# matchylabs/matchy

Measured on AMD Instinct MI355X. Metric: log GB/s scanned (matchy match hot path, 100K IoCs), higher is better.
Workload: dtype u8

## Files before the change

matchy_amd/csrc/db_image.cpp:

```cpp
#include "db_image.h"

#include <cstring>

namespace mxy {

namespace {
inline uint32_t rd32(const uint8_t* p) { uint32_t v; memcpy(&v, p, 4); return v; }
inline uint64_t rd64(const uint8_t* p) { uint64_t v; memcpy(&v, p, 8); return v; }

long find_metadata_marker(const uint8_t* d, size_t n) {
    static const uint8_t M[14] = {0xAB, 0xCD, 0xEF, 'M', 'a', 'x', 'M', 'i', 'n', 'd', '.', 'c', 'o', 'm'};
    if (n < 14) return -1;
    size_t start = n > 128 * 1024 ? n - 128 * 1024 : 0;
    long last = -1;
    for (size_t i = start; i + 14 <= n; ++i)
        if (memcmp(d + i, M, 14) == 0) last = (long)i;
    return last;
}
bool meta_uint(const DataValue& m, const char* key, uint64_t& out) {
    auto it = m.map.find(key);
    if (it == m.map.end()) return false;
    const DataValue& v = it->second;
    if (v.type != DataValue::UINT16 && v.type != DataValue::UINT32 && v.type != DataValue::UINT64) return false;
    out = v.u;
// ... 238 lines not shown
    }
    v4_start = 0;
    if (ip_version == 6) {
        uint32_t node = 0;
        for (int k = 0; k < 96; ++k) {
            uint32_t rec = out[node].x;
            if (rec < node_count) node = rec;
            else break;
        }
        v4_start = node;
    }
}

void DbImage::build_lit_table(std::vector<LitSlot>& slots, uint32_t& mask) const {
    const uint8_t* lh = bytes.data() + lh_off;
    size_t live = 0;
    for (uint32_t i = 0; i < lh_table_size; ++i) live += rd32(lh + lh_table_start + (size_t)i * 16 + 8) != 0xFFFFFFFFu;
    size_t cap = 16;
    while (cap < live * 2) cap <<= 1;
    mask = (uint32_t)(cap - 1);
    slots.assign(cap, LitSlot{0, 0xFFFFFFFFu, 0});
    for (uint32_t i = 0; i < lh_table_size; ++i) {
        const uint8_t* e = lh + lh_table_start + (size_t)i * 16;
        uint32_t so = rd32(e + 8);
        if (so == 0xFFFFFFFFu) continue;
        if ((size_t)so + 2 > lh_strings_size) continue;
        uint64_t h = rd64(e);
        uint32_t s = (uint32_t)(h ^ (h >> 32)) & mask;
        while (slots[s].str_off != 0xFFFFFFFFu) s = (s + 1) & mask;
        slots[s] = LitSlot{h, so, rd32(e + 12)};
    }
}

void DbImage::build_lit2pat(std::vector<uint32_t>& off, std::vector<uint32_t>& ids) const {
    off.assign(1, 0);
    ids.clear();
    if (!has_glob) return;
    const uint8_t* pg = bytes.data() + pg_off;
    uint32_t map_off = rd32(pg + 96), map_cnt = rd32(pg + 100);
    if (map_cnt == 0 || map_off == 0 || (size_t)map_off + 24 > pg_len) return;
    const uint8_t* a = pg + map_off;
    size_t alen = pg_len - map_off;
    if (memcmp(a, "ACLH", 4) != 0) return;
    uint32_t table_size = rd32(a + 12), pstart = rd32(a + 16);
    if (24 + (size_t)table_size * 16 > alen) return;
// ... 118 lines not shown
```

matchy_amd/csrc/engine.cpp:

```cpp
#include "engine.h"
#include "batch_reader.h"
#include "distinct.h"
#include "extract_render_core.h"
#include "render_core.h"
#include "tally.h"
#include "unicode_lower.h"

#include <dlfcn.h>

#include <algorithm>
#include <chrono>
#include <cstdio>
#include <cstdlib>
#include <cstring>
#include <stdexcept>
#include <unordered_set>

#include "domain_prefilter.h"
#include "hashes.h"

namespace mxy {

void check_launch(const char* kernel) {
    const hipError_t e = hipGetLastError();
// ... 239 lines not shown
            for (uint32_t wv : bm) set += (uint64_t)__builtin_popcount(wv);
            view.ip_bm24_permille = (uint32_t)(set * 1000 / ((uint64_t)bm.size() * 32));
            view.ip_bm24_any = set ? 1u : 0u;
        }
        bytes_uploaded += bm.size() * 4;
    }
    if (img.has_literal) {
        std::vector<LitSlot> slots;
        uint32_t mask;
        img.build_lit_table(slots, mask);
        lit_slots.upload(slots);
        const uint8_t* pool = img.bytes.data() + img.lh_off + img.lh_strings_offset;
        std::vector<uint8_t> pv(pool, pool + img.lh_strings_size);
        lit_pool.upload(pv);
        {
            size_t bits = (size_t)1 << 22;
            size_t live = 0;
            for (const LitSlot& sl : slots) live += sl.str_off != 0xFFFFFFFFu;
            while (bits < live * 64 && bits < ((size_t)1 << 31)) bits <<= 1;
            std::vector<uint32_t> bm(bits / 32, 0u);
            const uint32_t bmask = (uint32_t)(bits - 1);
            for (const LitSlot& sl : slots) {
                if (sl.str_off == 0xFFFFFFFFu || (size_t)sl.str_off + 2 > pv.size()) continue;
                const size_t kl = (size_t)pv[sl.str_off] | ((size_t)pv[sl.str_off + 1] << 8);
                if ((size_t)sl.str_off + 2 + kl > pv.size()) continue;
                uint64_t lane[4] = {0, 0, 0, 0};
                memcpy(lane, pv.data() + sl.str_off + 2, std::min<size_t>(kl, 32));
                const uint32_t b = name_hash31(lane[0], lane[1], lane[2], lane[3], (uint32_t)kl) & bmask;
                bm[b >> 5] |= 1u << (b & 31);
            }
            lit_bm.upload(bm);
            view.lit_bm = lit_bm.p; view.lit_bm_mask = bmask;
            bytes_uploaded += bm.size() * 4;
        }
        uint32_t max_len = 0;
        for (const LitSlot& sl : slots)
            if (sl.str_off != 0xFFFFFFFFu && (size_t)sl.str_off + 2 <= pv.size()) max_len = std::max<uint32_t>(max_len, (uint32_t)pv[sl.str_off] | ((uint32_t)pv[sl.str_off + 1] << 8));
        view.lit_max_len = max_len;
        view.lit_slots = lit_slots.p; view.lit_mask = mask; view.has_literal = 1;
        view.lit_pool = lit_pool.p; view.lit_pool_size = img.lh_strings_size;
        bytes_uploaded += slots.size() * sizeof(LitSlot) + pv.size();
    }
    if (img.has_glob) {
        const uint8_t* pgp = img.bytes.data() + img.pg_off;
        std::vector<uint8_t> pv(pgp, pgp + img.pg_len);
        pv.resize((pv.size() + 3) & ~(size_t)3, 0);
        pg.upload(pv);
        std::vector<uint32_t> off, ids;
        img.build_lit2pat(off, ids);
        if (ids.empty()) ids.push_back(0);
        lit2pat_off.upload(off);
        lit2pat.upload(ids);
// ... 782 lines not shown
            hh.n_cand_r = std::max(hh.n_cand_r, q.n_cand_r); hh.n_cand_d = std::max(hh.n_cand_d, q.n_cand_d);
            hh.n_dom = std::max(hh.n_dom, q.n_dom);
        }
        hint_ = hh;
    }
    const ScanCounters& c = host_counters_;
    if (c.error & 1) throw HipError{"scan: a candidate matches more than 65535 glob patterns (the hit record counts pattern ids in 16 bits)"};
    if (c.error & 4) throw HipError{"scan: a candidate is longer than 16 MiB (24-bit length field)"};
    if (trace) {
        ScanCounters t = host_slices_.p[0];
        for (int k = 1; k < ns; ++k) {
            const ScanCounters& s = host_slices_.p[k];
            t.n_dom += s.n_dom; t.n_rare += s.n_rare; t.n_rare_dom += s.n_rare_dom; t.n_tok += s.n_tok; t.n_heavy += s.n_heavy; t.n_cand_a += s.n_cand_a;
            t.n_cand += s.n_cand; t.n_hits += s.n_hits; t.n_ids += s.n_ids; t.n_glob_work += s.n_glob_work;
        }
        fprintf(stderr, "[matchy_amd] slices=%d lines=%llu n_dom=%u n_rare=%u+%u n_tok=%u n_heavy=%u n_cand=%u+%u (true %u) n_hits=%u (true %u) n_ids=%u glob_work=%u final=%u\n",
                ns, c.lines, t.n_dom, t.n_rare, t.n_rare_dom, t.n_tok, t.n_heavy, t.n_cand_a, t.n_cand, c.cand_true, t.n_hits, c.hits_true, t.n_ids, t.n_glob_work, c.n_final);
    }
    out.lines = c.lines; out.n_cand = single_ ? c.n_cand : c.cand_true;
    out.n_hits = !last_.lookup ? 0 : (single_ ? c.hits_true : c.n_final + (compact_ ? c.n_c4 : 0u));
    if (profile_) {
        MXY_HIP(hipEventElapsedTime(&timing_.anchor_ms, ev_[0], ev_[1]));
        if (last_forked_) {
            MXY_HIP(hipEventElapsedTime(&timing_.validate_ms, ev_[1], ev_[4]));
            timing_.rare_ms = 0; timing_.lookup_ms = 0;
        } else {
            MXY_HIP(hipEventElapsedTime(&timing_.validate_ms, ev_[1], ev_[2]));
            MXY_HIP(hipEventElapsedTime(&timing_.rare_ms, ev_[2], ev_[3]));
            MXY_HIP(hipEventElapsedTime(&timing_.lookup_ms, ev_[3], ev_[4]));
        }
        MXY_HIP(hipEventElapsedTime(&timing_.total_ms, ev_[0], ev_[4]));
        timing_.slices = ns;
// ... 584 lines not shown
```

matchy_amd/csrc/hashes.h:

```cpp
#pragma once
#include <cstddef>
#include <cstdint>

#if defined(__HIPCC__)
#include <hip/hip_runtime.h>
#define MXY_HD __host__ __device__ inline __attribute__((always_inline))
#else
#define MXY_HD inline
#endif

namespace mxy {

MXY_HD uint64_t rotl64(uint64_t x, int r) { return (x << r) | (x >> (64 - r)); }

template <class Fetch>
MXY_HD uint64_t xxh64_fetch(Fetch f, size_t len, uint64_t seed) {
    const uint64_t P1 = 11400714785074694791ULL, P2 = 14029467366897019727ULL, P3 = 1609587929392839161ULL,
                   P4 = 9650029242287828579ULL, P5 = 2870177450012600261ULL;
    auto rd64 = [&](size_t o) {
        uint64_t v = 0;
        for (int k = 7; k >= 0; --k) v = (v << 8) | (uint64_t)f(o + k);
        return v;
    };
    auto rd32 = [&](size_t o) {
// ... 117 lines not shown
};

MXY_HD uint32_t name_hash31(uint64_t l0, uint64_t l1, uint64_t l2, uint64_t l3, uint32_t n) {
    const uint64_t lane[4] = {l0, l1, l2, l3};
    uint32_t h = n * 0x9E3779B1u + 0x7F4A7C15u;
    for (int k = 0; k < 4; ++k) {
        const int rem = (int)n - 8 * k;
        const uint64_t m = rem >= 8 ? ~0ull : rem <= 0 ? 0ull : ((1ull << (8 * rem)) - 1ull);
        const uint64_t v = lane[k] & m;
        h = (h ^ (uint32_t)v) * 0x85EBCA6Bu; h ^= h >> 15;
        h = (h ^ (uint32_t)(v >> 32)) * 0xC2B2AE35u; h ^= h >> 13;
    }
    h *= 0x27D4EB2Fu; h ^= h >> 16;
    return h;
}

MXY_HD uint64_t fx_u32(uint32_t v) { return rotl64((uint64_t)v * 0xf1357aea2e62a9c5ULL, 26); }

constexpr uint32_t TLD_TAB_BITS = 11;
MXY_HD uint32_t tld_tab_slot(uint32_t lo, uint32_t hi24) { return ((lo ^ (hi24 * 0x9E3779B1u)) * 0x85EBCA6Bu) >> (32 - TLD_TAB_BITS); }

constexpr uint32_t TLD_PFX_BITS = 10;
constexpr uint32_t TLD_PFX_MAX_KEYS = (3u << TLD_PFX_BITS) / 4;
MXY_HD uint32_t tld_pfx_slot(uint32_t lo, uint32_t hi) { return ((lo ^ (hi * 0x9E3779B1u)) * 0x85EBCA6Bu) >> (32 - TLD_PFX_BITS); }

template <class Slot>
MXY_HD bool tld_pfx_has(const Slot* tab, uint32_t lo, uint32_t hi) {
    uint32_t slot = tld_pfx_slot(lo, hi);
    for (;;) {
        const Slot t = tab[slot];
// ... 29 lines not shown
```

matchy_amd/csrc/lookup_kernels.hip:

```cpp
#include <hip/hip_runtime.h>

#include <cstdlib>

#include "hashes.h"
#include "scan_types.h"

#include "device_shared.h"

namespace mxy {


__device__ __forceinline__ uint32_t d_utf8_decode(const uint8_t* s, uint32_t& cp) {
    const uint32_t c = s[0];
    if (c < 0x80) { cp = c; return 1; }
    if (c < 0xE0) { cp = ((c & 0x1Fu) << 6) | (s[1] & 0x3Fu); return 2; }
    if (c < 0xF0) { cp = ((c & 0x0Fu) << 12) | ((s[1] & 0x3Fu) << 6) | (s[2] & 0x3Fu); return 3; }
    cp = ((c & 0x07u) << 18) | ((s[1] & 0x3Fu) << 12) | ((s[2] & 0x3Fu) << 6) | (s[3] & 0x3Fu);
    return 4;
}
__device__ bool d_cp_in_ranges(const uint2* r, uint32_t n, uint32_t cp) {
    uint32_t lo = 0, hi = n;
    while (lo < hi) { const uint32_t mid = (lo + hi) >> 1; if (r[mid].y < cp) lo = mid + 1; else hi = mid; }
    return lo < n && r[lo].x <= cp;
}
// ... 38 lines not shown
                if (lo < db.lc_n && db.lc_map[lo * 3] == cp) {
                    const uint32_t e1 = db.lc_map[lo * 3 + 1];
                    np = e1 & 0xFF; pend = (uint64_t)(e1 >> 8) | ((uint64_t)db.lc_map[lo * 3 + 2] << 24);
                } else {
                    pend = 0; np = a;
                    for (uint32_t k = 0; k < a; ++k) pend |= (uint64_t)s[i + k] << (8 * k);
                }
            }
            i += a;
        }
        b = (uint32_t)pend & 0xFF; pend >>= 8; --np;
        return true;
    }
};

__device__ bool lit_lookup(const DevDb& db, const uint8_t* s0, uint32_t n0, uint32_t& pattern_id) {
    const uint8_t* s = s0;
    uint32_t n = n0;
    bool fold = false, stream = false;
    uint64_t h;
    if (db.ci) {
        uint64_t hi = 0;
        uint32_t k = 0;
        for (; k + 8 <= n0; k += 8) { uint64_t x; __builtin_memcpy(&x, s0 + k, 8); hi |= x; }
        for (; k < n0; ++k) hi |= s0[k];
        if ((hi & 0x8080808080808080ull) == 0) fold = true;
        else stream = true;
    }
    if (stream) {
        LowerStream ls(db, s0, n0);
        Xxh64Stream xs(0);
        uint32_t b;
        n = 0;
        while (ls.next(b)) {
            xs.push(b);
            if (++n > db.lit_max_len) return false;
        }
        h = xs.finish(0);
    } else {
        h = fold ? xxh64<true>(s, n, 0) : xxh64<false>(s, n, 0);
    }
    uint32_t slot = (uint32_t)(h ^ (h >> 32)) & db.lit_mask;
    for (;;) {
        LitSlot e = db.lit_slots[slot];
        if (e.str_off == 0xFFFFFFFFu) return false;
        if (e.hash == h) {
            const uint8_t* q = db.lit_pool + e.str_off;
            uint32_t sl = (uint32_t)q[0] | ((uint32_t)q[1] << 8);
            if (sl == n) {
                uint64_t diff = 0;
                if (stream) {
                    LowerStream ls(db, s0, n0);
                    uint32_t b, k = 0;
                    while (ls.next(b)) { diff |= (uint64_t)(q[2 + k] ^ b); ++k; }
                } else {
                    uint32_t k = 0;
                    for (; k + 8 <= n; k += 8) {
                        uint64_t x, y;
                        __builtin_memcpy(&x, q + 2 + k, 8);
                        __builtin_memcpy(&y, s + k, 8);
                        diff |= x ^ (fold ? ascii_lower8(y) : y);
                    }
                    if (k < n) {
                        if (n >= 8) {
                            uint64_t x, y;
                            __builtin_memcpy(&x, q + 2 + n - 8, 8);
                            __builtin_memcpy(&y, s + n - 8, 8);
                            diff |= x ^ (fold ? ascii_lower8(y) : y);
                        } else {
                            for (; k < n; ++k) diff |= (uint64_t)(q[2 + k] ^ (fold ? ascii_lower1(s[k]) : (uint32_t)s[k]));
                        }
                    }
                }
                if (diff == 0) { pattern_id = e.pattern_id; return true; }
            }
        }
        slot = (slot + 1) & db.lit_mask;
    }
}

__device__ __forceinline__ uint32_t ld32(const uint8_t* p) { return *reinterpret_cast<const uint32_t*>(p); }

__device__ uint32_t ac_transition(const uint8_t* ac, uint32_t ac_len, uint32_t node_off, uint32_t ch) {
    if (node_off + 20 > ac_len) return 0xFFFFFFFFu;
    uint32_t w0 = ld32(ac + node_off);
    uint32_t kind = w0 & 0xFF;
    if (kind == 1) return ((w0 >> 8) & 0xFF) == ch ? ld32(ac + node_off + 12) : 0xFFFFFFFFu;
    if (kind == 2) {
        uint32_t eo = ld32(ac + node_off + 12), cnt = (w0 >> 16) & 0xFF;
        if (eo + cnt * 8 > ac_len) return 0xFFFFFFFFu;
        for (uint32_t i = 0; i < cnt; ++i) {
            uint32_t ec = ac[eo + i * 8];
            if (ec == ch) return ld32(ac + eo + i * 8 + 4);
// ... 407 lines not shown
        }
        if (c.len_type != 0xFFFFFFFFu) {
            uint32_t type = c.len_type >> 24, tl = c.len_type & 0xFFFFFF;
            const uint8_t* text = p.log + c.start;
            h.cand = i; h.start = c.start; h.len_type = c.len_type;
            if (type == IT_IPV4) {
                uint32_t off, pfx;
                if (db.has_ip && trie_v4(db, c.v4, off, pfx)) { h.kind = 2; h.a = off; h.prefix_len = (uint8_t)pfx; emit = true; }
            } else if (type == IT_IPV6) {
                uint16_t seg[8];
                uint32_t off, pfx;
                if (db.has_ip && d_parse_ipv6(text, tl, seg) && trie_v6(db, seg, off, pfx)) { h.kind = 2; h.a = off; h.prefix_len = (uint8_t)pfx; emit = true; }
            } else {
                const bool alnum_tok = type == IT_MD5 || type == IT_SHA1 || type == IT_SHA256 || type == IT_SHA384 || type == IT_SHA512 ||
                                       type == IT_BITCOIN || type == IT_ETHEREUM || type == IT_MONERO;
                if (!db.ac_alnum && alnum_tok) c.pad = CAND_NO_GLOB;
                if (!GLOB && p.ac_filter && p.early_glob && c.pad == CAND_GLOB) {
                } else if (!GLOB && p.ac_filter && (c.pad == CAND_GLOB || (c.pad != CAND_NO_GLOB && (defer_unwalked || ac_touches_output(db, dv, text, tl))))) defer = true;
                else {
                    uint32_t pid = 0xFFFFFFFFu;
                    if (db.has_literal) { uint32_t q; if (lit_lookup(db, text, tl, q)) pid = q; }
                    if constexpr (GLOB) {
                        GlobSetList rs{globs};
                        StarStackFixed stk;
                        glob_find_all(db, dv, text_stage(p.log, p.len, c.start, tl, twin + threadIdx.x * GLOB_WIN_WORDS), outq + threadIdx.x * GLOB_OUTQ, rs, stk);
                        ng = rs.n;
                        spill = rs.over;
                    }
                    if (!spill && (pid != 0xFFFFFFFFu || ng)) { h.kind = 3; h.a = pid; h.n_globs = (uint16_t)ng; emit = true; }
                }
            }
        }
        if (p.direct && !GLOB) {
            if (emit) { pend[pn] = PendRec{h.start, h.len_type, h.a, (uint32_t)h.kind | ((uint32_t)h.prefix_len << 8)}; ++pn; }
            if (__ballot(pn == PEND_RECS)) { pack_pending(p.pk, pn, pend); pn = 0; }
        } else if (p.direct) {
// ... 42 lines not shown
    Hit SH{};
    SH.kind = 0xFF;
    for (uint32_t base = blockIdx.x * blockDim.x; base < n; base += stride) {
        const uint32_t k = base + threadIdx.x;
        Hit h{};
        bool emit = false;
        if (k < n) {
            const uint32_t tagged = p.spill[k], i = tagged & 0x7FFFFFFFu;
            const bool alt = (tagged >> 31) != 0;
            const Candidate c = alt ? (p.cands_alt && i < p.cand_alt_cap ? p.cands_alt[i] : Candidate{0, 0xFFFFFFFFu, 0, 0})
                                    : (i < p.cand_cap ? p.cands[i] : Candidate{0, 0xFFFFFFFFu, 0, 0});
            if (c.len_type != 0xFFFFFFFFu) {
                const uint32_t tl = c.len_type & 0xFFFFFF;
                h.cand = i; h.start = c.start; h.len_type = c.len_type;
                uint32_t pid = 0xFFFFFFFFu;
                if (db.has_literal) { uint32_t q; if (lit_lookup(db, p.log + c.start, tl, q)) pid = q; }
                for (uint32_t w = 0; w < bit_words; ++w) bits[w] = 0;
                GlobSetBitmap rs{bits, db.pattern_count};
                StarStackMem stk{bits + bit_words, (p.spill_words - bit_words) / 2};
                glob_find_all(db, dv, text_stage(p.log, p.len, c.start, tl, twin + threadIdx.x * GLOB_WIN_WORDS), outq + threadIdx.x * GLOB_OUTQ, rs, stk);
                uint32_t ng = rs.n;
                if (rs.over || ng > 0xFFFFu) { atomicOr(&p.counters->error, 1u); ng = 0; }
                if (ng) {
                    const uint32_t io = atomicAdd(&p.counters->n_ids, ng);
                    h.ids_off = io;
                    uint32_t o = io;
                    for (uint32_t w = 0; w < bit_words; ++w)
                        for (uint32_t m = bits[w]; m; m &= m - 1, ++o)
                            if (o < p.ids_cap) p.ids[o] = 32 * w + (uint32_t)__builtin_ctz(m);
                }
                if (pid != 0xFFFFFFFFu || ng) { h.kind = 3; h.a = pid; h.n_globs = (uint16_t)ng; emit = true; }
// ... 102 lines not shown
```

matchy_amd/csrc/scan_types.h:

```cpp
#pragma once
#include <hip/hip_runtime.h>

#include <cstdint>

namespace mxy {

enum ItemType : uint8_t {
    IT_DOMAIN = 0, IT_EMAIL = 1, IT_IPV4 = 2, IT_IPV6 = 3, IT_MD5 = 4, IT_SHA1 = 5, IT_SHA256 = 6,
    IT_SHA384 = 7, IT_SHA512 = 8, IT_BITCOIN = 9, IT_ETHEREUM = 10, IT_MONERO = 11, IT_COUNT = 12
};
enum ExtractFlags : uint32_t {
    EX_DOMAINS = 1, EX_EMAILS = 2, EX_IPV4 = 4, EX_IPV6 = 8, EX_HASHES = 16, EX_BITCOIN = 32, EX_ETHEREUM = 64,
    EX_MONERO = 128, EX_ALL = 255
};

struct Candidate {
    uint32_t start;
    uint32_t len_type;
    uint32_t v4;
    uint32_t pad;
};
constexpr uint32_t CAND_NO_GLOB = 1, CAND_GLOB = 2;

enum RareKind : uint32_t { RARE_V6 = 0, RARE_AT = 1, RARE_TOK = 2, HEAVY_B58 = 3, HEAVY_BECH32 = 4, HEAVY_ETH = 5, HEAVY_XMR = 6, RARE_DOM = 7 };
struct RareAnchor {
    uint32_t pos;
    uint32_t len_kind;
};

struct Hit {
    uint32_t cand;
    uint32_t a;
    uint32_t ids_off;
    uint16_t n_globs;
    uint8_t kind;
    uint8_t prefix_len;
    uint32_t start;
    uint32_t len_type;
};

struct LitSlot { uint64_t hash; uint32_t str_off; uint32_t pattern_id; };
struct PslSlot { uint64_t hash; uint32_t off; uint32_t len; };

struct DevDb {
    const uint2* ip_nodes;
    uint32_t ip_bm24_permille;
    uint32_t ip_bm24_any;
    const uint32_t* ip_bm24;
    const uint2* ip_l1;
    const uint2* ip_l24;
    const uint2* ip_leaf;
    uint32_t node_count;
    uint32_t ip_version;
    uint32_t v4_start_node;
    uint32_t has_ip;
    const LitSlot* lit_slots;
// ... 207 lines not shown
```

matchy_amd/csrc/validate_kernels.hip:

```cpp
#include <hip/hip_runtime.h>

#include <cstdlib>

#include "hashes.h"
#include "scan_types.h"

#include "device_shared.h"
#include "domain_planes.h"

namespace mxy {


struct BackReader {
    const uint8_t* p;
    uint32_t pos;
    uint32_t cb;
    uint32_t k;
    uint64_t cur, nxt;
    __device__ __forceinline__ static uint64_t load8(const uint8_t* a) { uint64_t v; __builtin_memcpy(&v, a, 8); return v; }
    __device__ __forceinline__ void init(const uint8_t* base, uint32_t q) {
        p = base; pos = q; cb = 0; k = 0; cur = 0; nxt = 0;
        if (q >= 16) { cb = q - 8; k = 8; cur = load8(p + cb); nxt = load8(p + cb - 8); }
    }
    __device__ __forceinline__ uint32_t next() {
// ... 761 lines not shown
    auto load_rec = [&](uint32_t i, Rec& r) {
        const uint32_t ic = i < nd ? i : 0u;
        const uint32_t j = p.dom_list[dom_plane_index(ic, 0)];
#pragma unroll
        for (int k = 0; k < 8; ++k) r.c[k] = p.dom_list[dom_plane_index(ic, 1 + k)];
        r.j = i < nd ? j : 0xFFFFFFFFu;
    };
    Rec cur, nxt;
    load_rec(blockIdx.x * blockDim.x + threadIdx.x, cur);
    {
        uint32_t g = cur.j;
#pragma unroll
        for (int k = 0; k < 8; ++k) g ^= cur.c[k];
        asm volatile("" ::"v"(g));
    }
    uint32_t pend_start = 0, pend_lt = 0, pend_word = 0xFFFFFFFFu, pend_bit = 0, n_valid = 0;
    uint32_t pend_sw[SFX ? 4 : 1] = {0}, pend_sb[SFX ? 4 : 1] = {0};
    bool pend = false, pend_over = false;
    uint32_t* sb = strbuf[threadIdx.x];
    auto queue_glob = [&](uint32_t b, uint32_t n) {
        if (!p.glob_work_d) return;
        const uint32_t lane = lane_id();
        const bool g = lane < n && b + lane < p.cand_cap && cw.buf[lane].pad == CAND_GLOB;
        const uint64_t m = __ballot(g);
        if (!m) return;
        uint32_t wb = 0;
        if (lane == 0) wb = atomicAdd(&p.counters->n_glob_work_d, (uint32_t)__popcll(m));
        wb = __builtin_amdgcn_readfirstlane(wb);
        const uint32_t slot = wb + mbcnt64(m);
        if (g && slot < p.glob_work_d_cap) p.glob_work_d[slot] = b + lane;
    };
    auto emit_pending = [&]() {
        if (!p.filter_lit) { cw_dense.append(pend, Candidate{pend_start, pend_lt, 0u, 0u}, p.cands, p.cand_cap, p.n_cand, SC); return; }
        bool lit = (pend_word >> pend_bit) & 1;
        uint32_t flag = 0;
        if constexpr (SFX) {
            bool g = pend_over;
#pragma unroll
            for (int q = 0; q < 4; ++q) g = g || ((pend_sw[q] >> pend_sb[q]) & 1);
            flag = g ? CAND_GLOB : CAND_NO_GLOB;
            lit = lit || g;
        }
        if constexpr (AC) flag = pend_over ? CAND_GLOB : CAND_NO_GLOB;
        if constexpr (AC || SFX) cw.append_then(pend && lit, Candidate{pend_start, pend_lt, 0u, flag}, p.cands, p.cand_cap, p.n_cand, queue_glob);
        else cw.append(pend && lit, Candidate{pend_start, pend_lt, 0u, flag}, p.cands, p.cand_cap, p.n_cand);
    };
    for (uint32_t base = blockIdx.x * blockDim.x; base < nd; base += stride) {
        const uint32_t i = base + threadIdx.x;
        emit_pending();
        pend = false;
        load_rec(i + stride, nxt);
        bool slow = false;
        if (cur.j != 0xFFFFFFFFu) {
            uint32_t s = 0, e = 0;
            int r = 2;
            if (!(cur.j & 0x80000000u)) r = domain_rules(tldtab, db.tld_pfx, p.min_labels, cur.j, cur.c, s, e);
            slow = r == 2;
            if (r == 1) {
                pend_start = s; pend_lt = (e - s) | ((uint32_t)IT_DOMAIN << 24); pend = true;
                pend_word = 0xFFFFFFFFu; pend_bit = 0;
                n_valid += 1;
                if (p.filter_lit) {
                    *reinterpret_cast<uint4*>(sb) = make_uint4(cur.c[0], cur.c[1], cur.c[2], cur.c[3]);
                    *reinterpret_cast<uint4*>(sb + 4) = make_uint4(cur.c[4], cur.c[5], cur.c[6], cur.c[7]);
                    const uint32_t o = 24 - (cur.j - s), n = e - s;
                    const uint32_t i0 = o >> 2, sh = o & 3;
                    uint32_t wd[9];
#pragma unroll
                    for (int k = 0; k < 9; ++k) wd[k] = (i0 + k) < 8 ? sb[(i0 + k) & 7] : 0u;
                    uint64_t ln[4];
#pragma unroll
                    for (int k = 0; k < 4; ++k)
                        ln[k] = (uint64_t)__builtin_amdgcn_alignbyte(wd[2 * k + 1], wd[2 * k], sh) |
                                ((uint64_t)__builtin_amdgcn_alignbyte(wd[2 * k + 2], wd[2 * k + 1], sh) << 32);
                    if (db.ci) {
#pragma unroll
                        for (int k = 0; k < 4; ++k) ln[k] = ascii_lower8(ln[k]);
                    }
                    const uint32_t b = name_hash31(ln[0], ln[1], ln[2], ln[3], n) & db.lit_bm_mask;
                    pend_word = db.lit_bm ? db.lit_bm[b >> 5] : 0u;
                    pend_bit = b & 31;
                    if constexpr (SFX) {
                        const uint64_t fb = 0x0101010101010101ull * db.sfx_first;
                        uint32_t M = 0;
#pragma unroll
                        for (int k = 0; k < 4; ++k) {
                            const uint64_t x = ln[k] ^ fb;
                            const uint64_t z = ~(((x & 0x7F7F7F7F7F7F7F7Full) + 0x7F7F7F7F7F7F7F7Full) | x) & 0x8080808080808080ull;
                            const uint32_t lo = (uint32_t)z >> 7, hi = (uint32_t)(z >> 32) >> 7;
                            M |= ((((lo * 0x01020408u) >> 24) & 0xFu) | ((((hi * 0x01020408u) >> 24) & 0xFu) << 4)) << (8 * k);
                        }
                        M &= n >= 32 ? 0xFFFFFFFFu : ((1u << n) - 1u);
                        pend_over = false;
                        uint32_t dm = db.sfx_dots;
#pragma unroll
                        for (int q = 0; q < 4; ++q) {
// ... 27 lines not shown
                            }
                        }
                    }
                    if constexpr (AC) {
                        uint32_t st = 0, any = 0;
#pragma unroll
                        for (int k = 0; k < 31; ++k) {
                            const uint32_t c = dcls[(uint32_t)(ln[k >> 3] >> (8 * (k & 7))) & 0xFF];
                            if ((uint32_t)k < n) {
                                const uint32_t t = st < dv.lds_states ? drows[st * db.dfa_k + c] : db.dfa[(size_t)st * db.dfa_k + c];
                                st = t & 0x7FFFFFFFu;
                                any |= t;
                            }
                        }
                        pend_over = (any >> 31) != 0;
                        if (pend_over) { pend_word = 0xFFFFFFFFu; pend_bit = 0; }
                    }
                }
            }
        }
        sw.append(slow, RareAnchor{cur.j & 0x7FFFFFFFu, (uint32_t)RARE_DOM}, p.rare_dom, p.rare_dom_cap, &p.counters->n_rare_dom);
        cur = nxt;
    }
    emit_pending();
    if constexpr (AC || SFX) cw.flush_then(p.cands, p.cand_cap, p.n_cand, queue_glob);
    else cw.flush(p.cands, p.cand_cap, p.n_cand);
    cw_dense.pad_rest(p.cands, p.cand_cap, SC);
    sw.flush(p.rare_dom, p.rare_dom_cap, &p.counters->n_rare_dom);
#pragma unroll
    for (int off = 32; off > 0; off >>= 1) n_valid += __shfl_down(n_valid, off);
    if (lane_id() == 0 && n_valid) atomicAdd(&p.counters->cand_true, n_valid);
}

__device__ __forceinline__ bool lit_bm_may_hit(const DevDb& db, const LogView& lg, uint32_t s, uint32_t n, bool ascii) {
    uint64_t l[4] = {0, 0, 0, 0};
    if (s + 32 <= lg.len) {
#pragma unroll
        for (int k = 0; k < 4; ++k) __builtin_memcpy(&l[k], lg.p + s + 8 * k, 8);
    } else {
        for (uint32_t k = 0; k < 32 && s + k < lg.len; ++k) l[k >> 3] |= (uint64_t)lg.p[s + k] << (8 * (k & 7));
    }
    if (db.ci) {
        if (!ascii) {
            if (n > 32) return true;
            uint64_t high = 0;
#pragma unroll
            for (int k = 0; k < 4; ++k) {
                const int rem = (int)n - 8 * k;
                const uint64_t m = rem >= 8 ? ~0ull : (rem <= 0 ? 0ull : ((1ull << (8 * rem)) - 1ull));
                high |= l[k] & m & 0x8080808080808080ull;
            }
            if (high) return true;
        }
#pragma unroll
        for (int k = 0; k < 4; ++k) l[k] = ascii_lower8(l[k]);
    }
    const uint32_t b = name_hash31(l[0], l[1], l[2], l[3], n) & db.lit_bm_mask;
    return ((db.lit_bm[b >> 5] >> (b & 31)) & 1u) != 0;
}

template <uint32_t VM>
__global__ __launch_bounds__(256) void k_validate(TokParams p, DevDb db) {
    constexpr bool MISC = (VM & 1u) != 0, DOM = (VM & 2u) != 0, TOK = (VM & 4u) != 0;
    __shared__ uint32_t bloom[DOM ? TLD_BLOOM_WORDS : 1];
    constexpr bool TLD_LDS = DOM && (MISC || TOK);
    __shared__ uint2 tldtab[TLD_LDS ? (1u << TLD_TAB_BITS) : 1];
    const uint2* const tldtab_p = TLD_LDS ? tldtab : db.tld_tab;
    constexpr uint32_t WIN = MISC ? 80 : 64;
    constexpr uint32_t WIN_BACK = WIN - (MISC ? 32 : 16);
    __shared__ __attribute__((aligned(16))) uint8_t winbuf[(MISC || DOM) ? 256 * WIN : 16];
    if constexpr (DOM && !MISC && !TOK) {
        if (blockIdx.x * blockDim.x >= min(p.counters->n_rare_dom, p.rare_dom_cap)) return;
    }
// ... 53 lines not shown
                        if (wide2) {
                            bool h2 = true;
#pragma unroll
                            for (int k = 0; k < 4; ++k) h2 = h2 & (((int)tl - 32 - 8 * k < 8) | (hex4((uint32_t)v2[k]) & hex4((uint32_t)(v2[k] >> 32))));
                            hex = h2;
                            if (hex && tl > 64) hex = all_hex_wide(s + 64, tl - 64);
                        } else {
                            hex = all_hex_wide(s + 32, tl - 32);
                        }
                    }
                    if (hex) {
                        c.start = ra.pos; c.len_type = tl | ((uint32_t)ht << 24); emit = true;
                        if (tok_filter) {
                            uint64_t l0 = w[0], l1 = w[1], l2 = w[2], l3 = w[3];
                            if (db.ci) { l0 = ascii_lower8(l0); l1 = ascii_lower8(l1); l2 = ascii_lower8(l2); l3 = ascii_lower8(l3); }
                            const uint32_t b = name_hash31(l0, l1, l2, l3, tl) & db.lit_bm_mask;
                            if (!((db.lit_bm[b >> 5] >> (b & 31)) & 1u)) { emit = false; ++unlisted_tok; }
                        }
                    }
                }
            }
            cw.append(emit, c, p.cands, p.cand_cap, p.n_cand);
        }
        {
            uint32_t hk = 0;
            if (live && (p.flags & EX_BITCOIN) && tl >= 26 && tl <= 62) {
                if (c0 == 'b' && c1 == 'c' && c2 == '1') hk = HEAVY_BECH32;
                else if (c0 == '1' || c0 == '3') {
                    auto has_byte = [](uint64_t x, uint32_t v) {
                        const uint64_t y = x ^ (0x0101010101010101ull * v);
                        return ~(((y & 0x7F7F7F7F7F7F7F7Full) + 0x7F7F7F7F7F7F7F7Full) | y) & 0x8080808080808080ull;
                    };
// ... 170 lines not shown
        }
        bool need_u8 = false;
        if (dr == WALK_LONG) dr = val_domain_resume(lg, db, p.min_labels, dl, ds, de, need_u8) ? WALK_YES : WALK_NO;
        for (uint64_t lm = __ballot(dr == WALK_YES && need_u8); lm; lm &= lm - 1) {
            const int src = __ffsll((long long)lm) - 1;
            const uint32_t us = (uint32_t)__shfl((int)ds, src), ue = (uint32_t)__shfl((int)de, src);
            const bool good = coop_valid_utf8(lg.p + us, ue - us);
            if ((int)lane_id() == src && !good) dr = WALK_NO;
        }
        if (dr == WALK_YES) {
            if (de - ds > 0xFFFFFFu) atomicOr(&p.counters->error, 4u);
            c.start = ds; c.len_type = (de - ds) | ((uint32_t)IT_DOMAIN << 24); emit = true;
        }
        if (lit_only && emit) {
            const uint32_t ty = c.len_type >> 24;
            if ((ty == IT_EMAIL || ty == IT_DOMAIN) && !lit_bm_may_hit(db, lg, c.start, c.len_type & 0xFFFFFFu, ty == IT_EMAIL)) { emit = false; ++unlisted; }
        }
        cw.append(emit, c, p.cands, p.cand_cap, p.n_cand);
    }
    }
    cw.flush(p.cands, p.cand_cap, p.n_cand);
#pragma unroll
    for (int off = 32; off > 0; off >>= 1) unlisted += __shfl_down(unlisted, off);
    if (lane_id() == 0 && cw.total + unlisted) atomicAdd(&p.counters->cand_true, cw.total + unlisted);
}

__global__ __launch_bounds__(64) void k_rare(TokParams p, DevDb db) {
    __shared__ __attribute__((aligned(16))) uint8_t tokbuf[64][112];
    __shared__ __attribute__((aligned(16))) uint8_t decbuf[64][96];
    LogView lg{p.log, p.len};
    __shared__ Candidate wb_cand[64];
// ... 63 lines not shown
```

Before: 2393.

## Reuse prefilter name hash for literal table lookup and use two-bit bloom filter

Rekeys the literal hash table on the 31-bit name hash that the scan kernels already compute for the bitmap prefilter. Candidates carry that hash and a CAND_HASHED flag, so the lookup stage skips the xxh64 rehash. Slots now also store the key length, which lets a probe reject a mismatch before comparing strings. The bitmap now sets two bits per key to cut false positives. The costs are extra host-side xxh64 verification when the table is built, and 31-bit hash collisions that must be resolved by string comparison.

```diff
diff --git a/matchy_amd/csrc/db_image.cpp b/matchy_amd/csrc/db_image.cpp
--- a/matchy_amd/csrc/db_image.cpp
+++ b/matchy_amd/csrc/db_image.cpp
@@ -276,21 +276,22 @@
 
 void DbImage::build_lit_table(std::vector<LitSlot>& slots, uint32_t& mask) const {
     const uint8_t* lh = bytes.data() + lh_off;
+    const uint8_t* pool = lh + lh_strings_offset;
+    auto key_len = [&](const uint8_t* e, uint32_t& so, uint32_t& kl) {
+        so = rd32(e + 8);
+        if (so == LIT_EMPTY || (size_t)so + 2 > lh_strings_size) return false;
+        kl = (uint32_t)pool[so] | ((uint32_t)pool[so + 1] << 8);
+        return (size_t)so + 2 + kl <= lh_strings_size && xxh64<false>(pool + so + 2, kl, 0) == rd64(e);
+    };
     size_t live = 0;
-    for (uint32_t i = 0; i < lh_table_size; ++i) live += rd32(lh + lh_table_start + (size_t)i * 16 + 8) != 0xFFFFFFFFu;
-    size_t cap = 16;
-    while (cap < live * 2) cap <<= 1;
+    uint32_t so, kl;
+    for (uint32_t i = 0; i < lh_table_size; ++i) live += key_len(lh + lh_table_start + (size_t)i * 16, so, kl);
+    const size_t cap = lit_table_capacity(live);
     mask = (uint32_t)(cap - 1);
-    slots.assign(cap, LitSlot{0, 0xFFFFFFFFu, 0});
+    slots.assign(cap, LitSlot{0, 0, LIT_EMPTY, 0});
     for (uint32_t i = 0; i < lh_table_size; ++i) {
         const uint8_t* e = lh + lh_table_start + (size_t)i * 16;
-        uint32_t so = rd32(e + 8);
-        if (so == 0xFFFFFFFFu) continue;
-        if ((size_t)so + 2 > lh_strings_size) continue;
-        uint64_t h = rd64(e);
-        uint32_t s = (uint32_t)(h ^ (h >> 32)) & mask;
-        while (slots[s].str_off != 0xFFFFFFFFu) s = (s + 1) & mask;
-        slots[s] = LitSlot{h, so, rd32(e + 12)};
+        if (key_len(e, so, kl)) lit_table_insert(slots, mask, pool, so, kl, rd32(e + 12));
     }
 }
 
diff --git a/matchy_amd/csrc/engine.cpp b/matchy_amd/csrc/engine.cpp
--- a/matchy_amd/csrc/engine.cpp
+++ b/matchy_amd/csrc/engine.cpp
@@ -277,28 +277,16 @@
         std::vector<uint8_t> pv(pool, pool + img.lh_strings_size);
         lit_pool.upload(pv);
         {
-            size_t bits = (size_t)1 << 22;
-            size_t live = 0;
-            for (const LitSlot& sl : slots) live += sl.str_off != 0xFFFFFFFFu;
-            while (bits < live * 64 && bits < ((size_t)1 << 31)) bits <<= 1;
-            std::vector<uint32_t> bm(bits / 32, 0u);
-            const uint32_t bmask = (uint32_t)(bits - 1);
-            for (const LitSlot& sl : slots) {
-                if (sl.str_off == 0xFFFFFFFFu || (size_t)sl.str_off + 2 > pv.size()) continue;
-                const size_t kl = (size_t)pv[sl.str_off] | ((size_t)pv[sl.str_off + 1] << 8);
-                if ((size_t)sl.str_off + 2 + kl > pv.size()) continue;
-                uint64_t lane[4] = {0, 0, 0, 0};
-                memcpy(lane, pv.data() + sl.str_off + 2, std::min<size_t>(kl, 32));
-                const uint32_t b = name_hash31(lane[0], lane[1], lane[2], lane[3], (uint32_t)kl) & bmask;
-                bm[b >> 5] |= 1u << (b & 31);
-            }
+            std::vector<uint32_t> bm;
+            uint32_t bmask;
+            lit_bitmap_build(slots, bm, bmask);
             lit_bm.upload(bm);
             view.lit_bm = lit_bm.p; view.lit_bm_mask = bmask;
             bytes_uploaded += bm.size() * 4;
         }
         uint32_t max_len = 0;
         for (const LitSlot& sl : slots)
-            if (sl.str_off != 0xFFFFFFFFu && (size_t)sl.str_off + 2 <= pv.size()) max_len = std::max<uint32_t>(max_len, (uint32_t)pv[sl.str_off] | ((uint32_t)pv[sl.str_off + 1] << 8));
+            if (sl.str_off != LIT_EMPTY) max_len = std::max(max_len, sl.len);
         view.lit_max_len = max_len;
         view.lit_slots = lit_slots.p; view.lit_mask = mask; view.has_literal = 1;
         view.lit_pool = lit_pool.p; view.lit_pool_size = img.lh_strings_size;
@@ -1111,8 +1099,10 @@
             t.n_dom += s.n_dom; t.n_rare += s.n_rare; t.n_rare_dom += s.n_rare_dom; t.n_tok += s.n_tok; t.n_heavy += s.n_heavy; t.n_cand_a += s.n_cand_a;
             t.n_cand += s.n_cand; t.n_hits += s.n_hits; t.n_ids += s.n_ids; t.n_glob_work += s.n_glob_work;
         }
-        fprintf(stderr, "[matchy_amd] slices=%d lines=%llu n_dom=%u n_rare=%u+%u n_tok=%u n_heavy=%u n_cand=%u+%u (true %u) n_hits=%u (true %u) n_ids=%u glob_work=%u final=%u\n",
-                ns, c.lines, t.n_dom, t.n_rare, t.n_rare_dom, t.n_tok, t.n_heavy, t.n_cand_a, t.n_cand, c.cand_true, t.n_hits, c.hits_true, t.n_ids, t.n_glob_work, c.n_final);
+        fprintf(stderr, "[matchy_amd] slices=%d lines=%llu n_dom=%u n_rare=%u+%u n_tok=%u n_heavy=%u n_cand=%u+%u (true %u) n_hits=%u (true %u) n_ids=%u glob_work=%u final=%u "
+                "cand_m=%u cand_d=%u cand_r=%u final_ids=%u c4=%u\n",
+                ns, c.lines, t.n_dom, t.n_rare, t.n_rare_dom, t.n_tok, t.n_heavy, t.n_cand_a, t.n_cand, c.cand_true, t.n_hits, c.hits_true, t.n_ids, t.n_glob_work, c.n_final,
+                c.n_cand_m, c.n_cand_d, c.n_cand_r, c.n_final_ids, c.n_c4);
     }
     out.lines = c.lines; out.n_cand = single_ ? c.n_cand : c.cand_true;
     out.n_hits = !last_.lookup ? 0 : (single_ ? c.hits_true : c.n_final + (compact_ ? c.n_c4 : 0u));
diff --git a/matchy_amd/csrc/hashes.h b/matchy_amd/csrc/hashes.h
--- a/matchy_amd/csrc/hashes.h
+++ b/matchy_amd/csrc/hashes.h
@@ -155,6 +155,17 @@
     h *= 0x27D4EB2Fu; h ^= h >> 16;
     return h;
 }
+inline uint32_t name_hash31_of(const uint8_t* s, size_t n) {
+    uint64_t lane[4] = {0, 0, 0, 0};
+    __builtin_memcpy(lane, s, n < 32 ? n : 32);
+    return name_hash31(lane[0], lane[1], lane[2], lane[3], (uint32_t)n);
+}
+
+MXY_HD uint32_t lit_bm_word(uint32_t h, uint32_t mask) { return (h & mask) >> 5; }
+MXY_HD uint32_t lit_bm_bits(uint32_t h) { return (1u << (h & 31)) | (1u << (h >> 27)); }
+MXY_HD bool lit_bm_pass(uint32_t word, uint32_t h) { return ((word >> (h & 31)) & (word >> (h >> 27)) & 1u) != 0; }
+
+MXY_HD uint32_t lit_home(uint32_t h, uint32_t mask) { return h & mask; }
 
 MXY_HD uint64_t fx_u32(uint32_t v) { return rotl64((uint64_t)v * 0xf1357aea2e62a9c5ULL, 26); }
 
diff --git a/matchy_amd/csrc/lit_table.h b/matchy_amd/csrc/lit_table.h
--- /dev/null
+++ b/matchy_amd/csrc/lit_table.h
@@ -0,0 +1,47 @@
+#pragma once
+#include <cstddef>
+#include <cstdint>
+#include <vector>
+
+#include "hashes.h"
+
+namespace mxy {
+
+constexpr uint32_t LIT_EMPTY = 0xFFFFFFFFu;
+struct alignas(16) LitSlot { uint32_t hash; uint32_t len; uint32_t str_off; uint32_t pattern_id; };
+
+inline size_t lit_table_capacity(size_t live) {
+    size_t cap = 16;
+    while (cap < live * 2) cap <<= 1;
+    return cap;
+}
+
+inline void lit_table_insert(std::vector<LitSlot>& slots, uint32_t mask, const uint8_t* pool, uint32_t str_off, uint32_t len, uint32_t pattern_id) {
+    const uint32_t h = name_hash31_of(pool + str_off + 2, len);
+    uint32_t s = lit_home(h, mask);
+    while (slots[s].str_off != LIT_EMPTY) s = (s + 1) & mask;
+    slots[s] = LitSlot{h, len, str_off, pattern_id};
+}
+
+inline void lit_bitmap_build(const std::vector<LitSlot>& slots, std::vector<uint32_t>& bm, uint32_t& bmask, size_t min_bits = (size_t)1 << 22) {
+    size_t bits = min_bits, live = 0;
+    for (const LitSlot& sl : slots) live += sl.str_off != LIT_EMPTY;
+    while (bits < live * 64 && bits < ((size_t)1 << 31)) bits <<= 1;
+    bm.assign(bits / 32, 0u);
+    bmask = (uint32_t)(bits - 1);
+    for (const LitSlot& sl : slots)
+        if (sl.str_off != LIT_EMPTY) bm[lit_bm_word(sl.hash, bmask)] |= lit_bm_bits(sl.hash);
+}
+
+template <class SameKey>
+MXY_HD bool lit_probe(const LitSlot* slots, uint32_t mask, uint32_t h, uint32_t n, SameKey same_key, uint32_t& pattern_id) {
+    uint32_t slot = lit_home(h, mask);
+    for (;;) {
+        const LitSlot e = slots[slot];
+        if (e.str_off == LIT_EMPTY) return false;
+        if (e.hash == h && e.len == n && same_key(e.str_off)) { pattern_id = e.pattern_id; return true; }
+        slot = (slot + 1) & mask;
+    }
+}
+
+}
diff --git a/matchy_amd/csrc/lookup_kernels.hip b/matchy_amd/csrc/lookup_kernels.hip
--- a/matchy_amd/csrc/lookup_kernels.hip
+++ b/matchy_amd/csrc/lookup_kernels.hip
@@ -76,69 +76,70 @@
     }
 };
 
-__device__ bool lit_lookup(const DevDb& db, const uint8_t* s0, uint32_t n0, uint32_t& pattern_id) {
-    const uint8_t* s = s0;
-    uint32_t n = n0;
-    bool fold = false, stream = false;
-    uint64_t h;
-    if (db.ci) {
-        uint64_t hi = 0;
-        uint32_t k = 0;
-        for (; k + 8 <= n0; k += 8) { uint64_t x; __builtin_memcpy(&x, s0 + k, 8); hi |= x; }
-        for (; k < n0; ++k) hi |= s0[k];
-        if ((hi & 0x8080808080808080ull) == 0) fold = true;
-        else stream = true;
-    }
-    if (stream) {
-        LowerStream ls(db, s0, n0);
-        Xxh64Stream xs(0);
-        uint32_t b;
-        n = 0;
-        while (ls.next(b)) {
-            xs.push(b);
-            if (++n > db.lit_max_len) return false;
-        }
-        h = xs.finish(0);
-    } else {
-        h = fold ? xxh64<true>(s, n, 0) : xxh64<false>(s, n, 0);
-    }
-    uint32_t slot = (uint32_t)(h ^ (h >> 32)) & db.lit_mask;
-    for (;;) {
-        LitSlot e = db.lit_slots[slot];
-        if (e.str_off == 0xFFFFFFFFu) return false;
-        if (e.hash == h) {
-            const uint8_t* q = db.lit_pool + e.str_off;
-            uint32_t sl = (uint32_t)q[0] | ((uint32_t)q[1] << 8);
-            if (sl == n) {
-                uint64_t diff = 0;
-                if (stream) {
-                    LowerStream ls(db, s0, n0);
-                    uint32_t b, k = 0;
-                    while (ls.next(b)) { diff |= (uint64_t)(q[2 + k] ^ b); ++k; }
+__device__ bool lit_lookup(const DevDb& db, const uint8_t* s, uint32_t n0, uint32_t cand_hash, bool hashed, uint32_t& pattern_id) {
+    uint32_t n = n0, h = cand_hash;
+    bool fold = db.ci != 0, stream = false;
+    if (!hashed) {
+        if (db.ci) {
+            uint64_t hi = 0;
+            uint32_t k = 0;
+            for (; k + 8 <= n0; k += 8) { uint64_t x; __builtin_memcpy(&x, s + k, 8); hi |= x; }
+            for (; k < n0; ++k) hi |= s[k];
+            if ((hi & 0x8080808080808080ull) != 0) { fold = false; stream = true; }
+        }
+        uint64_t l0 = 0, l1 = 0, l2 = 0, l3 = 0;
+        if (stream) {
+            LowerStream ls(db, s, n0);
+            uint32_t b;
+            n = 0;
+            while (ls.next(b)) {
+                const uint64_t v = (uint64_t)b << (8 * (n & 7));
+                const uint32_t k = n >> 3;
+                l0 |= k == 0 ? v : 0; l1 |= k == 1 ? v : 0; l2 |= k == 2 ? v : 0; l3 |= k == 3 ? v : 0;
+                if (++n > db.lit_max_len) return false;
+            }
+        } else if (n >= 8) {
+            auto lane = [&](uint32_t o) {
+                uint64_t v = 0;
+                if (o + 8 <= n) __builtin_memcpy(&v, s + o, 8);
+                else if (o < n) { __builtin_memcpy(&v, s + n - 8, 8); v >>= 8 * (8 - (n - o)); }
+                return v;
+            };
+            l0 = lane(0); l1 = lane(8); l2 = lane(16); l3 = lane(24);
+        } else {
+            for (uint32_t k = 0; k < n; ++k) l0 |= (uint64_t)s[k] << (8 * k);
+        }
+        if (fold) { l0 = ascii_lower8(l0); l1 = ascii_lower8(l1); l2 = ascii_lower8(l2); l3 = ascii_lower8(l3); }
+        h = name_hash31(l0, l1, l2, l3, n);
+    }
+    return lit_probe(db.lit_slots, db.lit_mask, h, n, [&](uint32_t str_off) {
+        const uint8_t* q = db.lit_pool + str_off + 2;
+        uint64_t diff = 0;
+        if (stream) {
+            LowerStream ls(db, s, n0);
+            uint32_t b, k = 0;
+            while (ls.next(b)) { diff |= (uint64_t)(q[k] ^ b); ++k; }
+        } else {
+            uint32_t k = 0;
+            for (; k + 8 <= n; k += 8) {
+                uint64_t x, y;
+                __builtin_memcpy(&x, q + k, 8);
+                __builtin_memcpy(&y, s + k, 8);
+                diff |= x ^ (fold ? ascii_lower8(y) : y);
+            }
+            if (k < n) {
+                if (n >= 8) {
+                    uint64_t x, y;
+                    __builtin_memcpy(&x, q + n - 8, 8);
+                    __builtin_memcpy(&y, s + n - 8, 8);
+                    diff |= x ^ (fold ? ascii_lower8(y) : y);
                 } else {
-                    uint32_t k = 0;
-                    for (; k + 8 <= n; k += 8) {
-                        uint64_t x, y;
-                        __builtin_memcpy(&x, q + 2 + k, 8);
-                        __builtin_memcpy(&y, s + k, 8);
-                        diff |= x ^ (fold ? ascii_lower8(y) : y);
-                    }
-                    if (k < n) {
-                        if (n >= 8) {
-                            uint64_t x, y;
-                            __builtin_memcpy(&x, q + 2 + n - 8, 8);
-                            __builtin_memcpy(&y, s + n - 8, 8);
-                            diff |= x ^ (fold ? ascii_lower8(y) : y);
-                        } else {
-                            for (; k < n; ++k) diff |= (uint64_t)(q[2 + k] ^ (fold ? ascii_lower1(s[k]) : (uint32_t)s[k]));
-                        }
-                    }
+                    for (; k < n; ++k) diff |= (uint64_t)(q[k] ^ (fold ? ascii_lower1(s[k]) : (uint32_t)s[k]));
                 }
-                if (diff == 0) { pattern_id = e.pattern_id; return true; }
-            }
-        }
-        slot = (slot + 1) & db.lit_mask;
-    }
+            }
+        }
+        return diff == 0;
+    }, pattern_id);
 }
 
 __device__ __forceinline__ uint32_t ld32(const uint8_t* p) { return *reinterpret_cast<const uint32_t*>(p); }
@@ -576,12 +577,12 @@
             } else {
                 const bool alnum_tok = type == IT_MD5 || type == IT_SHA1 || type == IT_SHA256 || type == IT_SHA384 || type == IT_SHA512 ||
                                        type == IT_BITCOIN || type == IT_ETHEREUM || type == IT_MONERO;
-                if (!db.ac_alnum && alnum_tok) c.pad = CAND_NO_GLOB;
-                if (!GLOB && p.ac_filter && p.early_glob && c.pad == CAND_GLOB) {
-                } else if (!GLOB && p.ac_filter && (c.pad == CAND_GLOB || (c.pad != CAND_NO_GLOB && (defer_unwalked || ac_touches_output(db, dv, text, tl))))) defer = true;
+                const uint32_t known = (!db.ac_alnum && alnum_tok) ? CAND_NO_GLOB : (c.pad & CAND_GLOB_MASK);
+                if (!GLOB && p.ac_filter && p.early_glob && known == CAND_GLOB) {
+                } else if (!GLOB && p.ac_filter && (known == CAND_GLOB || (known != CAND_NO_GLOB && (defer_unwalked || ac_touches_output(db, dv, text, tl))))) defer = true;
                 else {
                     uint32_t pid = 0xFFFFFFFFu;
-                    if (db.has_literal) { uint32_t q; if (lit_lookup(db, text, tl, q)) pid = q; }
+                    if (db.has_literal) { uint32_t q; if (lit_lookup(db, text, tl, c.v4, (c.pad & CAND_HASHED) != 0, q)) pid = q; }
                     if constexpr (GLOB) {
                         GlobSetList rs{globs};
                         StarStackFixed stk;
@@ -654,7 +655,7 @@
                 const uint32_t tl = c.len_type & 0xFFFFFF;
                 h.cand = i; h.start = c.start; h.len_type = c.len_type;
                 uint32_t pid = 0xFFFFFFFFu;
-                if (db.has_literal) { uint32_t q; if (lit_lookup(db, p.log + c.start, tl, q)) pid = q; }
+                if (db.has_literal) { uint32_t q; if (lit_lookup(db, p.log + c.start, tl, c.v4, (c.pad & CAND_HASHED) != 0, q)) pid = q; }
                 for (uint32_t w = 0; w < bit_words; ++w) bits[w] = 0;
                 GlobSetBitmap rs{bits, db.pattern_count};
                 StarStackMem stk{bits + bit_words, (p.spill_words - bit_words) / 2};
diff --git a/matchy_amd/csrc/scan_types.h b/matchy_amd/csrc/scan_types.h
--- a/matchy_amd/csrc/scan_types.h
+++ b/matchy_amd/csrc/scan_types.h
@@ -2,6 +2,8 @@
 #include <hip/hip_runtime.h>
 
 #include <cstdint>
+
+#include "lit_table.h"
 
 namespace mxy {
 
@@ -20,7 +22,7 @@
     uint32_t v4;
     uint32_t pad;
 };
-constexpr uint32_t CAND_NO_GLOB = 1, CAND_GLOB = 2;
+constexpr uint32_t CAND_NO_GLOB = 1, CAND_GLOB = 2, CAND_GLOB_MASK = 3, CAND_HASHED = 4;
 
 enum RareKind : uint32_t { RARE_V6 = 0, RARE_AT = 1, RARE_TOK = 2, HEAVY_B58 = 3, HEAVY_BECH32 = 4, HEAVY_ETH = 5, HEAVY_XMR = 6, RARE_DOM = 7 };
 struct RareAnchor {
@@ -39,7 +41,6 @@
     uint32_t len_type;
 };
 
-struct LitSlot { uint64_t hash; uint32_t str_off; uint32_t pattern_id; };
 struct PslSlot { uint64_t hash; uint32_t off; uint32_t len; };
 
 struct DevDb {
diff --git a/matchy_amd/csrc/validate_kernels.hip b/matchy_amd/csrc/validate_kernels.hip
--- a/matchy_amd/csrc/validate_kernels.hip
+++ b/matchy_amd/csrc/validate_kernels.hip
@@ -799,14 +799,14 @@
         for (int k = 0; k < 8; ++k) g ^= cur.c[k];
         asm volatile("" ::"v"(g));
     }
-    uint32_t pend_start = 0, pend_lt = 0, pend_word = 0xFFFFFFFFu, pend_bit = 0, n_valid = 0;
+    uint32_t pend_start = 0, pend_lt = 0, pend_word = 0xFFFFFFFFu, pend_hash = 0, n_valid = 0;
     uint32_t pend_sw[SFX ? 4 : 1] = {0}, pend_sb[SFX ? 4 : 1] = {0};
     bool pend = false, pend_over = false;
     uint32_t* sb = strbuf[threadIdx.x];
     auto queue_glob = [&](uint32_t b, uint32_t n) {
         if (!p.glob_work_d) return;
         const uint32_t lane = lane_id();
-        const bool g = lane < n && b + lane < p.cand_cap && cw.buf[lane].pad == CAND_GLOB;
+        const bool g = lane < n && b + lane < p.cand_cap && (cw.buf[lane].pad & CAND_GLOB_MASK) == CAND_GLOB;
         const uint64_t m = __ballot(g);
         if (!m) return;
         uint32_t wb = 0;
@@ -817,7 +817,7 @@
     };
     auto emit_pending = [&]() {
         if (!p.filter_lit) { cw_dense.append(pend, Candidate{pend_start, pend_lt, 0u, 0u}, p.cands, p.cand_cap, p.n_cand, SC); return; }
-        bool lit = (pend_word >> pend_bit) & 1;
+        bool lit = lit_bm_pass(pend_word, pend_hash);
         uint32_t flag = 0;
         if constexpr (SFX) {
             bool g = pend_over;
@@ -827,8 +827,8 @@
             lit = lit || g;
         }
         if constexpr (AC) flag = pend_over ? CAND_GLOB : CAND_NO_GLOB;
-        if constexpr (AC || SFX) cw.append_then(pend && lit, Candidate{pend_start, pend_lt, 0u, flag}, p.cands, p.cand_cap, p.n_cand, queue_glob);
-        else cw.append(pend && lit, Candidate{pend_start, pend_lt, 0u, flag}, p.cands, p.cand_cap, p.n_cand);
+        if constexpr (AC || SFX) cw.append_then(pend && lit, Candidate{pend_start, pend_lt, pend_hash, flag | CAND_HASHED}, p.cands, p.cand_cap, p.n_cand, queue_glob);
+        else cw.append(pend && lit, Candidate{pend_start, pend_lt, pend_hash, flag | CAND_HASHED}, p.cands, p.cand_cap, p.n_cand);
     };
     for (uint32_t base = blockIdx.x * blockDim.x; base < nd; base += stride) {
         const uint32_t i = base + threadIdx.x;
@@ -843,7 +843,7 @@
             slow = r == 2;
             if (r == 1) {
                 pend_start = s; pend_lt = (e - s) | ((uint32_t)IT_DOMAIN << 24); pend = true;
-                pend_word = 0xFFFFFFFFu; pend_bit = 0;
+                pend_word = 0xFFFFFFFFu; pend_hash = 0;
                 n_valid += 1;
                 if (p.filter_lit) {
                     *reinterpret_cast<uint4*>(sb) = make_uint4(cur.c[0], cur.c[1], cur.c[2], cur.c[3]);
@@ -862,9 +862,8 @@
 #pragma unroll
                         for (int k = 0; k < 4; ++k) ln[k] = ascii_lower8(ln[k]);
                     }
-                    const uint32_t b = name_hash31(ln[0], ln[1], ln[2], ln[3], n) & db.lit_bm_mask;
-                    pend_word = db.lit_bm ? db.lit_bm[b >> 5] : 0u;
-                    pend_bit = b & 31;
+                    pend_hash = name_hash31(ln[0], ln[1], ln[2], ln[3], n);
+                    pend_word = db.lit_bm ? db.lit_bm[lit_bm_word(pend_hash, db.lit_bm_mask)] : 0u;
                     if constexpr (SFX) {
                         const uint64_t fb = 0x0101010101010101ull * db.sfx_first;
                         uint32_t M = 0;
@@ -922,7 +921,7 @@
                             }
                         }
                         pend_over = (any >> 31) != 0;
-                        if (pend_over) { pend_word = 0xFFFFFFFFu; pend_bit = 0; }
+                        if (pend_over) pend_word = 0xFFFFFFFFu;
                     }
                 }
             }
@@ -940,7 +939,8 @@
     if (lane_id() == 0 && n_valid) atomicAdd(&p.counters->cand_true, n_valid);
 }
 
-__device__ __forceinline__ bool lit_bm_may_hit(const DevDb& db, const LogView& lg, uint32_t s, uint32_t n, bool ascii) {
+__device__ __forceinline__ bool lit_bm_may_hit(const DevDb& db, const LogView& lg, uint32_t s, uint32_t n, bool ascii, bool& hashed, uint32_t& h) {
+    hashed = false;
     uint64_t l[4] = {0, 0, 0, 0};
     if (s + 32 <= lg.len) {
 #pragma unroll
@@ -963,8 +963,9 @@
 #pragma unroll
         for (int k = 0; k < 4; ++k) l[k] = ascii_lower8(l[k]);
     }
-    const uint32_t b = name_hash31(l[0], l[1], l[2], l[3], n) & db.lit_bm_mask;
-    return ((db.lit_bm[b >> 5] >> (b & 31)) & 1u) != 0;
+    h = name_hash31(l[0], l[1], l[2], l[3], n);
+    hashed = true;
+    return lit_bm_pass(db.lit_bm[lit_bm_word(h, db.lit_bm_mask)], h);
 }
 
 template <uint32_t VM>
@@ -1048,8 +1049,8 @@
                         if (tok_filter) {
                             uint64_t l0 = w[0], l1 = w[1], l2 = w[2], l3 = w[3];
                             if (db.ci) { l0 = ascii_lower8(l0); l1 = ascii_lower8(l1); l2 = ascii_lower8(l2); l3 = ascii_lower8(l3); }
-                            const uint32_t b = name_hash31(l0, l1, l2, l3, tl) & db.lit_bm_mask;
-                            if (!((db.lit_bm[b >> 5] >> (b & 31)) & 1u)) { emit = false; ++unlisted_tok; }
+                            c.v4 = name_hash31(l0, l1, l2, l3, tl); c.pad = CAND_HASHED;
+                            if (!lit_bm_pass(db.lit_bm[lit_bm_word(c.v4, db.lit_bm_mask)], c.v4)) { emit = false; ++unlisted_tok; }
                         }
                     }
                 }
@@ -1250,7 +1251,12 @@
         }
         if (lit_only && emit) {
             const uint32_t ty = c.len_type >> 24;
-            if ((ty == IT_EMAIL || ty == IT_DOMAIN) && !lit_bm_may_hit(db, lg, c.start, c.len_type & 0xFFFFFFu, ty == IT_EMAIL)) { emit = false; ++unlisted; }
+            if (ty == IT_EMAIL || ty == IT_DOMAIN) {
+                bool hashed;
+                uint32_t h;
+                if (!lit_bm_may_hit(db, lg, c.start, c.len_type & 0xFFFFFFu, ty == IT_EMAIL, hashed, h)) { emit = false; ++unlisted; }
+                else if (hashed) { c.v4 = h; c.pad |= CAND_HASHED; }
+            }
         }
         cw.append(emit, c, p.cands, p.cand_cap, p.n_cand);
     }
```

After: 2395, median of 6. Within noise of the previous version (+0.1%).
